# PaddlePaddle/PaddleScience

Measured on NVIDIA H100. Metric: collocation-points/sec PDE residual loss+grad (LDC N-S), higher is better.
Workload: dtype f32

## Files before the change

paddlescience_b200/csrc/kernels_wgmma.cuh:

```cuda
#pragma once

#include "kernels_thin.cuh"

#ifndef PPSCI_EMUL
#include <stdint.h>

namespace ppsci {
namespace wg {

constexpr int KCH = 32;
constexpr int THREADS = 256;
constexpr int TM = 64;
constexpr int A_TILE_BYTES = TM * KCH * 4;
__host__ __device__ inline int tile_points(int C) { return TM / C; }

__host__ __device__ inline int stage_bytes(int N) { return 2 * A_TILE_BYTES + 2 * N * KCH * 4; }
__host__ __device__ inline int fwd_smem_bytes(int N) { return 2 * stage_bytes(N) + 1024 + 64; }
constexpr int PREFETCH_MAX_CS = 8;

__host__ __device__ __forceinline__ uint32_t sw128(int row, int kk) {
  return (uint32_t)(row * 128 + ((((kk >> 2) ^ row) & 7) << 4) + ((kk & 3) << 2));
}
__device__ __forceinline__ uint32_t sw128_q(int row, int kq) { return (uint32_t)(row * 128 + (((kq ^ row) & 7) << 4)); }

__device__ __forceinline__ uint32_t smem_u32(const void* p) { return (uint32_t)__cvta_generic_to_shared(p); }

__device__ __forceinline__ float tf32_rn(float x) {
  uint32_t u;
  asm("cvt.rna.tf32.f32 %0, %1;" : "=r"(u) : "f"(x));
  return __uint_as_float(u);
}

__device__ __forceinline__ void mbar_init(uint32_t bar, uint32_t count) {
  asm volatile("mbarrier.init.shared::cta.b64 [%0], %1;" ::"r"(bar), "r"(count) : "memory");
}
__device__ __forceinline__ void mbar_expect_tx(uint32_t bar, uint32_t bytes) {
  asm volatile("mbarrier.arrive.expect_tx.shared::cta.b64 _, [%0], %1;" ::"r"(bar), "r"(bytes) : "memory");
}
__device__ __forceinline__ bool mbar_try_wait(uint32_t bar, uint32_t parity) {
  uint32_t ok;
  asm volatile(
      "{\n\t.reg .pred p;\n\t"
      "mbarrier.try_wait.parity.shared::cta.b64 p, [%1], %2;\n\t"
      "selp.u32 %0, 1, 0, p;\n\t}"
      : "=r"(ok)
      : "r"(bar), "r"(parity)
      : "memory");
  return ok != 0;
}
__device__ __forceinline__ void mbar_wait(uint32_t bar, uint32_t parity) {
  uint32_t spins = 0;
  while (!mbar_try_wait(bar, parity)) {
    if (++spins > (1u << 26)) __trap();
  }
}
__device__ __forceinline__ void bulk_g2s(uint32_t dst_smem, const void* src, uint32_t bytes, uint32_t bar) {
  asm volatile("cp.async.bulk.shared::cluster.global.mbarrier::complete_tx::bytes [%0], [%1], %2, [%3];" ::"r"(dst_smem),
               "l"(src), "r"(bytes), "r"(bar)
               : "memory");
}
__device__ __forceinline__ void fence_proxy_async() { asm volatile("fence.proxy.async.shared::cta;" ::: "memory"); }

__device__ __forceinline__ uint64_t make_desc(uint32_t saddr) {
  uint64_t d = 0;
  d |= (uint64_t)((saddr & 0x3FFFFu) >> 4);
  d |= (uint64_t)1 << 16;
  d |= (uint64_t)(1024 >> 4) << 32;
  d |= (uint64_t)1 << 62;
  return d;
}
__device__ __forceinline__ void wgmma_fence() { asm volatile("wgmma.fence.sync.aligned;" ::: "memory"); }
__device__ __forceinline__ void wgmma_commit() { asm volatile("wgmma.commit_group.sync.aligned;" ::: "memory"); }
template <int N>
__device__ __forceinline__ void wgmma_wait() {
  asm volatile("wgmma.wait_group.sync.aligned %0;" ::"n"(N) : "memory");
}
#define WG_T0 "%0, %1, %2, %3, %4, %5, %6, %7"
#define WG_T1 WG_T0 ", %8, %9, %10, %11, %12, %13, %14, %15"
#define WG_T2 WG_T1 ", %16, %17, %18, %19, %20, %21, %22, %23"
#define WG_T3 WG_T2 ", %24, %25, %26, %27, %28, %29, %30, %31"
#define WG_T4 WG_T3 ", %32, %33, %34, %35, %36, %37, %38, %39"
#define WG_T5 WG_T4 ", %40, %41, %42, %43, %44, %45, %46, %47"
#define WG_T6 WG_T5 ", %48, %49, %50, %51, %52, %53, %54, %55"
#define WG_T7 WG_T6 ", %56, %57, %58, %59, %60, %61, %62, %63"
#define WG_O8(b) "+f"(d[b]), "+f"(d[b + 1]), "+f"(d[b + 2]), "+f"(d[b + 3]), "+f"(d[b + 4]), "+f"(d[b + 5]), "+f"(d[b + 6]), "+f"(d[b + 7])
#define WG_O0 WG_O8(0)
#define WG_O1 WG_O0, WG_O8(8)
#define WG_O2 WG_O1, WG_O8(16)
#define WG_O3 WG_O2, WG_O8(24)
#define WG_O4 WG_O3, WG_O8(32)
#define WG_O5 WG_O4, WG_O8(40)
#define WG_O6 WG_O5, WG_O8(48)
#define WG_O7 WG_O6, WG_O8(56)
#define WG_MMA(M, G, IA, IB, IP)                                                                                  \
  __device__ __forceinline__ void wgmma_tf32(float (&d)[M / 2], uint64_t da, uint64_t db, uint32_t accumulate) { \
    asm volatile(                                                                                                 \
        "{\n\t.reg .pred p;\n\t"                                                                                  \
        "setp.ne.b32 p, %" #IP ", 0;\n\t"                                                                          \
        "wgmma.mma_async.sync.aligned.m64n" #M "k8.f32.tf32.tf32 {" WG_T##G "}, %" #IA ", %" #IB ", p, 1, 1;\n\t}"  \
        : WG_O##G                                                                                                 \
        : "l"(da), "l"(db), "r"(accumulate));                                                                     \
  }
WG_MMA(16, 0, 8, 9, 10)
WG_MMA(32, 1, 16, 17, 18)
WG_MMA(48, 2, 24, 25, 26)
WG_MMA(64, 3, 32, 33, 34)
WG_MMA(80, 4, 40, 41, 42)
WG_MMA(96, 5, 48, 49, 50)
WG_MMA(112, 6, 56, 57, 58)
WG_MMA(128, 7, 64, 65, 66)
#undef WG_MMA

__global__ void k_wg_prep_w(const float* __restrict__ W, float* __restrict__ img, int K, int N, int transposed) {
  const long long i = (long long)blockIdx.x * blockDim.x + threadIdx.x;
  if (i >= (long long)K * N) return;
  const int n = (int)(i / K), k = (int)(i % K);
  const float w = transposed ? W[(long long)n * K + k] : W[(long long)k * N + n];
  const float hi = tf32_rn(w);
  float* blk = img + (long long)(k / KCH) * 2 * N * KCH;
  const uint32_t off = sw128(n, k % KCH) >> 2;
  blk[off] = hi;
  blk[(long long)N * KCH + off] = w - hi;
}

struct WgArgs {
  AOperand<float> A;
  JetLayout J;
  const float* Wimg;
  int Kdim;
  int Kvalid;
  int Nout;
  const float* bias;
  float* Out;
  int ldo;
  long long oplane;
  long long Np;
  int num_tiles;
  const float* Zprev;
  int ldz;
  long long zplane;
  int act;
};

__device__ __forceinline__ unsigned char* xchg(unsigned char* base_ptr, int sbytes, int N, int r, int col) {
  return base_ptr + sbytes + 2 * A_TILE_BYTES + r * N * 4 + ((((col >> 2) ^ r) & 7) << 4) + (((col >> 2) & ~7) << 4) +
         (col & 3) * 4;
}

template <class L, int NQ, bool DX>
__global__ void __launch_bounds__(THREADS, 1) k_wg_layer(WgArgs g) {
  PPSCI_DYN_SMEM(smem_dyn);
  const uint32_t base = (smem_u32(smem_dyn) + 1023u) & ~1023u;
  unsigned char* base_ptr = smem_dyn + (base - smem_u32(smem_dyn));
  constexpr int CS = L::CS;
  constexpr int TP = TM / CS;
  constexpr int rows_used = CS * TP;
  constexpr int PPR = (THREADS / 32) * 4;
  constexpr int MAXI = (TP + PPR - 1) / PPR;
  constexpr int N = NQ * 32;
  constexpr int NH = N / 2;
  constexpr bool PREFETCH = CS <= PREFETCH_MAX_CS;
  const int sbytes = stage_bytes(N);
  const uint32_t bar0 = base + 2 * sbytes;
  const uint32_t b_bytes = (uint32_t)(2 * N * KCH * 4);
  const int tid = threadIdx.x, warp = tid >> 5, lane = tid & 31, wgi = tid >> 7;
  const int kq = lane & 7, psub = lane >> 3;
  const int nchunks = g.Kdim / KCH;
  const int act = g.A.act;

  if (tid == 0) {
    mbar_init(bar0, 1);
    mbar_init(bar0 + 8, 1);
    asm volatile("fence.mbarrier_init.release.cluster;" ::: "memory");
  }
  for (int s = 0; s < 2; ++s) {
    float4* az = reinterpret_cast<float4*>(base_ptr + s * sbytes);
    for (int i = tid; i < 2 * A_TILE_BYTES / 16; i += THREADS) az[i] = make_float4(0.f, 0.f, 0.f, 0.f);
  }
  fence_proxy_async();
  __syncthreads();

  float4 z[MAXI][CS];
  bool zok[MAXI];
  auto load_z = [&](int tile, int j) {
#pragma unroll
    for (int i = 0; i < MAXI; ++i) {
      const int pl = warp * 4 + psub + i * PPR;
      const long long p = (long long)tile * TP + pl;
      zok[i] = pl < TP && tile < g.num_tiles && p < g.Np;
      if (g.Kvalid && j * KCH + 4 * kq >= g.Kvalid) zok[i] = false;
      const float* src = g.A.Z + p * g.A.ld + j * KCH + 4 * kq;
#pragma unroll
      for (int c = 0; c < CS; ++c)
        z[i][c] = zok[i] ? __ldg(reinterpret_cast<const float4*>(src + (long long)c * g.A.plane)) : make_float4(0.f, 0.f, 0.f, 0.f);
    }
  };
  if constexpr (PREFETCH) load_z(blockIdx.x, 0);

  float ex[NH / 2], cr[NH / 2];
  const int rbase = (warp & 3) * 16 + (lane >> 2);
  const int cbase = wgi * NH + 2 * (lane & 3);
  uint32_t it = 0;
  for (int tile = blockIdx.x; tile < g.num_tiles; tile += gridDim.x) {
    const long long p0 = (long long)tile * TP;
#pragma unroll
    for (int e = 0; e < NH / 2; ++e) ex[e] = cr[e] = 0.f;
    for (int j = 0; j < nchunks; ++j, ++it) {
      const uint32_t s = it & 1u;
      wgmma_wait<1>();
      __syncthreads();
      const uint32_t st_addr = base + s * sbytes;
      unsigned char* st_ptr = base_ptr + s * sbytes;
      if (tid == 0) {
        mbar_expect_tx(bar0 + 8 * s, b_bytes);
        bulk_g2s(st_addr + 2 * A_TILE_BYTES, g.Wimg + (long long)j * 2 * N * KCH, b_bytes, bar0 + 8 * s);
      }
      if constexpr (!PREFETCH) load_z(tile, j);
#pragma unroll
      for (int i = 0; i < MAXI; ++i) {
        const int pl = warp * 4 + psub + i * PPR;
        if (pl >= TP) continue;
        const bool valid = zok[i];
        float yout[CS][4];
        if constexpr (DX) {
#pragma unroll
          for (int c = 0; c < CS; ++c) {
            yout[c][0] = z[i][c].x; yout[c][1] = z[i][c].y; yout[c][2] = z[i][c].z; yout[c][3] = z[i][c].w;
          }
        } else {
#pragma unroll
          for (int t = 0; t < 4; ++t) {
            auto comp = [&](const float4& v) { return t == 0 ? v.x : t == 1 ? v.y : t == 2 ? v.z : v.w; };
            float sc[6];
            float y0;
            act_coef<float, L::KM>(act, comp(z[i][0]), y0, sc);
            yout[0][t] = valid ? y0 : 0.f;
            jet_fwd<float, L>(g.J, sc, [&](int c) { return comp(z[i][c]); }, [&](int c, float v) { yout[c][t] = valid ? v : 0.f; });
          }
        }
#pragma unroll
        for (int c = 0; c < CS; ++c) {
          float4 h, l;
          h.x = tf32_rn(yout[c][0]); h.y = tf32_rn(yout[c][1]); h.z = tf32_rn(yout[c][2]); h.w = tf32_rn(yout[c][3]);
          l.x = yout[c][0] - h.x; l.y = yout[c][1] - h.y; l.z = yout[c][2] - h.z; l.w = yout[c][3] - h.w;
          const uint32_t off = sw128_q(c * TP + pl, kq);
          *reinterpret_cast<float4*>(st_ptr + off) = h;
          *reinterpret_cast<float4*>(st_ptr + A_TILE_BYTES + off) = l;
        }
      }
      if constexpr (PREFETCH) {
        if (j + 1 < nchunks) load_z(tile, j + 1);
        else load_z(tile + gridDim.x, 0);
      }
      fence_proxy_async();
      __syncthreads();
      mbar_wait(bar0 + 8 * s, (it >> 1) & 1u);
      const uint64_t a_hi = make_desc(st_addr), a_lo = make_desc(st_addr + A_TILE_BYTES);
      const uint64_t b_hi = make_desc(st_addr + 2 * A_TILE_BYTES + wgi * NH * 128), b_lo = b_hi + (uint64_t)(N * 128 / 16);
      wgmma_fence();
#pragma unroll
      for (int ks = 0; ks < KCH / 8; ++ks) {
        const uint64_t inc = (uint64_t)(2 * ks);
        const uint32_t first = (j == 0 && ks == 0) ? 0u : 1u;
        wgmma_tf32(ex, a_hi + inc, b_hi + inc, first);
        wgmma_tf32(cr, a_lo + inc, b_hi + inc, first);
        wgmma_tf32(cr, a_hi + inc, b_lo + inc, 1u);
      }
      wgmma_commit();
    }
    wgmma_wait<0>();
    if constexpr (!DX) {
#pragma unroll
      for (int h = 0; h < 2; ++h) {
        const int r = rbase + 8 * h;
        const int c = r / TP, pl = r - c * TP;
        const long long p = p0 + pl;
        if (r >= rows_used || p >= g.Np) continue;
        float* out_row = g.Out + (long long)c * g.oplane + p * g.ldo;
#pragma unroll
        for (int j = 0; j < NH / 8; ++j) {
          const int col = cbase + 8 * j;
          float2 v = make_float2(ex[4 * j + 2 * h] + cr[4 * j + 2 * h], ex[4 * j + 2 * h + 1] + cr[4 * j + 2 * h + 1]);
          if (c == 0 && g.bias) {
            v.x += __ldg(g.bias + col);
            v.y += __ldg(g.bias + col + 1);
          }
          *reinterpret_cast<float2*>(out_row + col) = v;
        }
      }
    } else {
      __syncthreads();
#pragma unroll
      for (int h = 0; h < 2; ++h) {
        const int r = rbase + 8 * h;
#pragma unroll
        for (int j = 0; j < NH / 8; ++j)
          *reinterpret_cast<float2*>(xchg(base_ptr, sbytes, N, r, cbase + 8 * j)) =
              make_float2(ex[4 * j + 2 * h] + cr[4 * j + 2 * h], ex[4 * j + 2 * h + 1] + cr[4 * j + 2 * h + 1]);
      }
      constexpr int N4 = N / 4;
      auto load_zc = [&](int item, float4 (&zc)[CS]) {
        const int pl = item / N4, q = item - pl * N4;
        const long long p = p0 + pl;
        if (item >= TP * N4 || p >= g.Np) return;
#pragma unroll
        for (int c = 0; c < CS; ++c)
          zc[c] = __ldg(reinterpret_cast<const float4*>(g.Zprev + (long long)c * g.zplane + p * g.ldz + 4 * q));
      };
      float4 znext[CS];
      if constexpr (PREFETCH) load_zc(tid, znext);
      __syncthreads();
      for (int item = tid; item < TP * N4; item += THREADS) {
        const int pl = item / N4, q = item - pl * N4;
        const long long p = p0 + pl;
        float4 zc[CS];
        if constexpr (PREFETCH) {
#pragma unroll
          for (int c = 0; c < CS; ++c) zc[c] = znext[c];
          load_zc(item + THREADS, znext);
        } else {
          load_zc(item, zc);
        }
        if (p >= g.Np) continue;
        float4 xc[CS];
#pragma unroll
        for (int c = 0; c < CS; ++c) xc[c] = *reinterpret_cast<const float4*>(xchg(base_ptr, sbytes, N, c * TP + pl, 4 * q));
        float ob[CS][4];
#pragma unroll
        for (int t = 0; t < 4; ++t) {
          auto comp = [&](const float4& v) { return t == 0 ? v.x : t == 1 ? v.y : t == 2 ? v.z : v.w; };
          float sc[6];
          float y0;
          act_coef<float, L::KM + 1>(g.act, comp(zc[0]), y0, sc);
          ob[0][t] = jet_adj<float, L>(g.J, sc, [&](int c) { return comp(zc[c]); }, [&](int c) { return comp(xc[c]); },
                                       [&](int c, float v) { ob[c][t] = v; });
        }
        float* out = g.Out + p * g.ldo + 4 * q;
#pragma unroll
        for (int c = 0; c < CS; ++c)
          *reinterpret_cast<float4*>(out + (long long)c * g.oplane) = make_float4(ob[c][0], ob[c][1], ob[c][2], ob[c][3]);
      }
      fence_proxy_async();
      __syncthreads();
    }
  }
}

__host__ __device__ constexpr int dw_pch(int C) { return C >= 8 ? 4 : C >= 3 ? 8 : 32 / C; }
__host__ __device__ constexpr int dw_groups(int C) { return dw_pch(C) / 4 * C; }
__host__ __device__ constexpr int dw_ksteps(int C) { return (dw_groups(C) + 1) / 2; }
__host__ __device__ constexpr int dw_atoms(int C) { return (dw_ksteps(C) + 3) / 4; }
__host__ __device__ constexpr int dw_maxq(int C) { return C <= 5 ? 4 : C <= 8 ? 2 : 1; }
__host__ __device__ constexpr int dw_smem_bytes(int C, int bnq) {
  return 2 * 2 * dw_atoms(C) * bnq * 32 * 128 + bnq * 32 * 4 + dw_pch(C) / 4 * 2 * C * 256 * 4 + bnq * 32 * 2 * 256 + 1024;
}
constexpr int DW_TK = 128;
constexpr int DW_FLUSH_ROWS = 512;
__host__ __device__ constexpr int dw_flush(int C) {
  return DW_FLUSH_ROWS / (dw_pch(C) * C) > 1 ? DW_FLUSH_ROWS / (dw_pch(C) * C) : 1;
}

struct WgDwArgs {
  AOperand<float> A;
  JetLayout J;
  const float* Zbar;
  int ldzb;
  long long zbplane;
  int Kdim;
  int Nout;
  int col_blocks;
  float* dW;
  float* db;
  long long Np;
  int chunks_per_split;
};

__device__ __forceinline__ void wgmma_tf32_rA_m64n64(float (&d)[32], const uint32_t (&a)[4], uint64_t db) {
  asm volatile(
      "{\n\t.reg .pred p;\n\t"
      "setp.ne.b32 p, %37, 0;\n\t"
      "wgmma.mma_async.sync.aligned.m64n64k8.f32.tf32.tf32 "
      "{%0, %1, %2, %3, %4, %5, %6, %7, %8, %9, %10, %11, %12, %13, %14, %15, "
      "%16, %17, %18, %19, %20, %21, %22, %23, %24, %25, %26, %27, %28, %29, %30, %31}, "
      "{%32, %33, %34, %35}, %36, p, 1, 1;\n\t}"
      : "+f"(d[0]), "+f"(d[1]), "+f"(d[2]), "+f"(d[3]), "+f"(d[4]), "+f"(d[5]), "+f"(d[6]), "+f"(d[7]), "+f"(d[8]),
        "+f"(d[9]), "+f"(d[10]), "+f"(d[11]), "+f"(d[12]), "+f"(d[13]), "+f"(d[14]), "+f"(d[15]), "+f"(d[16]),
        "+f"(d[17]), "+f"(d[18]), "+f"(d[19]), "+f"(d[20]), "+f"(d[21]), "+f"(d[22]), "+f"(d[23]), "+f"(d[24]),
        "+f"(d[25]), "+f"(d[26]), "+f"(d[27]), "+f"(d[28]), "+f"(d[29]), "+f"(d[30]), "+f"(d[31])
      : "r"(a[0]), "r"(a[1]), "r"(a[2]), "r"(a[3]), "l"(db), "r"(1u));
}
__device__ __forceinline__ void wgmma_tf32_rA_m64n32(float (&d)[16], const uint32_t (&a)[4], uint64_t db) {
  asm volatile(
      "{\n\t.reg .pred p;\n\t"
      "setp.ne.b32 p, %21, 0;\n\t"
      "wgmma.mma_async.sync.aligned.m64n32k8.f32.tf32.tf32 "
      "{%0, %1, %2, %3, %4, %5, %6, %7, %8, %9, %10, %11, %12, %13, %14, %15}, "
      "{%16, %17, %18, %19}, %20, p, 1, 1;\n\t}"
      : "+f"(d[0]), "+f"(d[1]), "+f"(d[2]), "+f"(d[3]), "+f"(d[4]), "+f"(d[5]), "+f"(d[6]), "+f"(d[7]), "+f"(d[8]),
        "+f"(d[9]), "+f"(d[10]), "+f"(d[11]), "+f"(d[12]), "+f"(d[13]), "+f"(d[14]), "+f"(d[15])
      : "r"(a[0]), "r"(a[1]), "r"(a[2]), "r"(a[3]), "l"(db), "r"(1u));
}

template <class L, int BNQ>
__global__ void __launch_bounds__(THREADS, 1) k_wg_dw(WgDwArgs g) {
  PPSCI_DYN_SMEM(smem_dyn);
  const uint32_t base = (smem_u32(smem_dyn) + 1023u) & ~1023u;
  unsigned char* base_ptr = smem_dyn + (base - smem_u32(smem_dyn));
  constexpr int CS = L::CS, PCH = dw_pch(CS), QPC = PCH / 4, G = dw_groups(CS), KS = dw_ksteps(CS), NA = dw_atoms(CS);
  constexpr int BN = BNQ * 32, NB = BNQ / 2, TAIL = BNQ & 1;
  constexpr int ATOM = BN * 128;
  constexpr int STAGE = 2 * NA * ATOM;
  constexpr int BI = (G * BN + THREADS - 1) / THREADS;
  const int tid = threadIdx.x, warp = tid >> 5, lane = tid & 31, wgi = tid >> 7, t = lane & 3;
  const int kb = blockIdx.x / g.col_blocks, n0 = (blockIdx.x - kb * g.col_blocks) * BN;
  const int Np = (int)g.Np;
  const int total_chunks = (Np + PCH - 1) / PCH;
  const int ch_begin = blockIdx.y * g.chunks_per_split;
  const int ch_end = ch_begin + g.chunks_per_split < total_chunks ? ch_begin + g.chunks_per_split : total_chunks;
  if (ch_begin >= ch_end) return;
  const int act = g.A.act;
  const int krow = kb * DW_TK + wgi * 64 + (warp & 3) * 16 + (lane >> 2);

  float* bsum = reinterpret_cast<float*>(base_ptr + 2 * STAGE);
  for (int i = tid; i < (2 * STAGE + BN * 4) / 16; i += THREADS)
    reinterpret_cast<float4*>(base_ptr)[i] = make_float4(0.f, 0.f, 0.f, 0.f);
  __syncthreads();

  float ex[NB > 0 ? NB : 1][32], ext[TAIL ? 16 : 1], cr[NB > 0 ? NB : 1][32], crt[TAIL ? 16 : 1];
#pragma unroll
  for (int nb = 0; nb < NB; ++nb)
#pragma unroll
    for (int i = 0; i < 32; ++i) ex[nb][i] = cr[nb][i] = 0.f;
#pragma unroll
  for (int i = 0; i < (TAIL ? 16 : 1); ++i) ext[i] = crt[i] = 0.f;

  auto acc_at = [&](int e) -> float {
    return e < 32 * NB ? ex[e >> 5][e & 31] + cr[e >> 5][e & 31] : ext[e - 32 * NB] + crt[e - 32 * NB];
  };
  float4* part = reinterpret_cast<float4*>(base_ptr + 2 * STAGE + BN * 4 + QPC * 2 * CS * THREADS * 4);
#pragma unroll
  for (int q = 0; q < BN / 8; ++q) part[q * THREADS + tid] = make_float4(0.f, 0.f, 0.f, 0.f);
  auto flush = [&]() {
#pragma unroll
    for (int q = 0; q < BN / 8; ++q) {
      float4 p = part[q * THREADS + tid];
      p.x += acc_at(4 * q); p.y += acc_at(4 * q + 1); p.z += acc_at(4 * q + 2); p.w += acc_at(4 * q + 3);
      part[q * THREADS + tid] = p;
    }
#pragma unroll
    for (int nb = 0; nb < NB; ++nb)
#pragma unroll
      for (int i = 0; i < 32; ++i) ex[nb][i] = cr[nb][i] = 0.f;
#pragma unroll
    for (int i = 0; i < (TAIL ? 16 : 1); ++i) ext[i] = crt[i] = 0.f;
  };

  float* za = reinterpret_cast<float*>(base_ptr + 2 * STAGE + BN * 4);
  auto za_at = [&](int qq, int h, int c) -> float* { return za + ((qq * 2 + h) * CS + c) * THREADS + tid; };
  float4 zb[BI];
  auto load_a = [&](int ch) {
    const int p0 = ch * PCH;
#pragma unroll
    for (int qq = 0; qq < QPC; ++qq)
#pragma unroll
      for (int h = 0; h < 2; ++h) {
        const int p = p0 + 4 * qq + t;
        const int k = krow + 8 * h;
        const bool ok = p < Np && k < g.Kdim;
        const float* src = g.A.Z + (ok ? (long long)p * g.A.ld + k : 0);
#pragma unroll
        for (int c = 0; c < CS; ++c)
          asm volatile("cp.async.ca.shared.global [%0], [%1], 4, %2;" ::"r"(smem_u32(za_at(qq, h, c))),
                       "l"(src + (ok ? (long long)c * g.A.plane : 0)), "r"(ok ? 4 : 0)
                       : "memory");
      }
    asm volatile("cp.async.commit_group;" ::: "memory");
  };
  auto load_b = [&](int ch) {
    const int p0 = ch * PCH;
#pragma unroll
    for (int i = 0; i < BI; ++i) {
      const int item = tid + THREADS * i;
      const int gi = item / BN, n = item - gi * BN;
      const int qq = gi / CS, c = gi - qq * CS;
      const int p = p0 + 4 * qq;
      const bool ok = item < G * BN && n0 + n < g.Nout;
      const float* src = g.Zbar + (long long)c * g.zbplane + (long long)p * g.ldzb + n0 + n;
      zb[i].x = ok && p < Np ? __ldg(src) : 0.f;
      zb[i].y = ok && p + 1 < Np ? __ldg(src + g.ldzb) : 0.f;
      zb[i].z = ok && p + 2 < Np ? __ldg(src + 2 * g.ldzb) : 0.f;
      zb[i].w = ok && p + 3 < Np ? __ldg(src + 3 * g.ldzb) : 0.f;
    }
  };

  load_a(ch_begin);
  load_b(ch_begin);
  uint32_t ahi[KS][4], alo[KS][4];
  for (int ch = ch_begin; ch < ch_end; ++ch) {
    const int sidx = (ch - ch_begin) & 1;
    const uint32_t st_addr = base + sidx * STAGE;
    unsigned char* st = base_ptr + sidx * STAGE;
#pragma unroll
    for (int i = 0; i < BI; ++i) {
      const int item = tid + THREADS * i;
      if (item >= G * BN) continue;
      const int gi = item / BN, n = item - gi * BN;
      const float4 v = zb[i];
      float4 hi, lo;
      hi.x = tf32_rn(v.x); hi.y = tf32_rn(v.y); hi.z = tf32_rn(v.z); hi.w = tf32_rn(v.w);
      lo.x = v.x - hi.x; lo.y = v.y - hi.y; lo.z = v.z - hi.z; lo.w = v.w - hi.w;
      const uint32_t off = (gi >> 3) * ATOM + sw128_q(n, gi & 7);
      *reinterpret_cast<float4*>(st + off) = hi;
      *reinterpret_cast<float4*>(st + NA * ATOM + off) = lo;
      if (kb == 0 && gi % CS == 0) atomicAdd(bsum + n, (v.x + v.y) + (v.z + v.w));
    }
    wgmma_wait<0>();
    if (ch > ch_begin && (ch - ch_begin) % dw_flush(CS) == 0) flush();
    asm volatile("cp.async.wait_group 0;" ::: "memory");
    float av[QPC][2][CS];
#pragma unroll
    for (int qq = 0; qq < QPC; ++qq)
#pragma unroll
      for (int h = 0; h < 2; ++h) {
        float z[CS], sc[6];
#pragma unroll
        for (int c = 0; c < CS; ++c) z[c] = *za_at(qq, h, c);
        act_coef<float, L::KM>(act, z[0], av[qq][h][0], sc);
        jet_fwd<float, L>(g.J, sc, [&](int c) { return z[c]; }, [&](int c, float v) { av[qq][h][c] = v; });
      }
    if (ch + 1 < ch_end) load_a(ch + 1);
    fence_proxy_async();
    __syncthreads();
    if (ch + 1 < ch_end) load_b(ch + 1);
#pragma unroll
    for (int s = 0; s < KS; ++s)
#pragma unroll
      for (int e = 0; e < 2; ++e)
#pragma unroll
        for (int h = 0; h < 2; ++h) {
          const int gi = 2 * s + e;
          const float v = gi < G ? av[gi / CS][h][gi % CS] : 0.f;
          const float vh = tf32_rn(v);
          ahi[s][2 * e + h] = __float_as_uint(vh);
          alo[s][2 * e + h] = __float_as_uint(v - vh);
        }
    wgmma_fence();
#pragma unroll
    for (int s = 0; s < KS; ++s) {
      const uint64_t b_hi = make_desc(st_addr + (s >> 2) * ATOM + (s & 3) * 32);
      const uint64_t b_lo = b_hi + (uint64_t)(NA * ATOM / 16);
#pragma unroll
      for (int nb = 0; nb < NB; ++nb) {
        const uint64_t bo = (uint64_t)(nb * 64 * 128 / 16);
        wgmma_tf32_rA_m64n64(ex[nb], ahi[s], b_hi + bo);
        wgmma_tf32_rA_m64n64(cr[nb], alo[s], b_hi + bo);
        wgmma_tf32_rA_m64n64(cr[nb], ahi[s], b_lo + bo);
      }
      if constexpr (TAIL) {
        const uint64_t bo = (uint64_t)(NB * 64 * 128 / 16);
        wgmma_tf32_rA_m64n32(ext, ahi[s], b_hi + bo);
        wgmma_tf32_rA_m64n32(crt, alo[s], b_hi + bo);
        wgmma_tf32_rA_m64n32(crt, ahi[s], b_lo + bo);
      }
    }
    wgmma_commit();
  }
  wgmma_wait<0>();
#pragma unroll
  for (int h = 0; h < 2; ++h) {
    const int k = krow + 8 * h;
    if (k >= g.Kdim) continue;
    float* row = g.dW + (long long)k * g.Nout + n0;
#pragma unroll
    for (int j = 0; j < BN / 8; ++j) {
      if (n0 + 8 * j >= g.Nout) break;
      const int col = 8 * j + 2 * t;
      const float4 p = part[j * THREADS + tid];
      atomicAdd(row + col, (h ? p.z : p.x) + acc_at(4 * j + 2 * h));
      atomicAdd(row + col + 1, (h ? p.w : p.y) + acc_at(4 * j + 2 * h + 1));
    }
  }
  if (kb == 0) {
    __syncthreads();
    if (tid < BN && n0 + tid < g.Nout) atomicAdd(g.db + n0 + tid, bsum[tid]);
  }
}

}

inline int wg_kpad(int K) { return (K + wg::KCH - 1) / wg::KCH * wg::KCH; }
inline bool wg_shape_ok(int K, int N) { return K % wg::KCH == 0 && K >= 32 && K <= 1024 && N % 32 == 0 && N >= 32 && N <= 256; }
inline bool wg_plan_ok(const ppsci_plan_spec& s, const JetLayout& J) {
  return s.dtype == PPSCI_F32 && !s.gated && !act_has_param(s.act) && with_lay(WgLays{}, J, [](auto) {});
}
inline bool wg_fwd_ok(const ppsci_plan_spec& s, int l) {
  if (l == 1) return s.dense_in && s.n_layers >= 2 && s.widths[0] % 4 == 0 && wg_shape_ok(wg_kpad(s.widths[0]), s.widths[1]);
  if (l < 2 || l > s.n_layers) return false;
  return wg_shape_ok(s.widths[l - 1], s.widths[l]);
}
inline bool wg_dx_ok(const ppsci_plan_spec& s, int l) {
  if (l < 2 || l > s.n_layers) return false;
  return wg_shape_ok(s.widths[l], s.widths[l - 1]);
}

inline bool wg_dw_ok(const ppsci_plan_spec& s, int l) {
  if (l < 1 || (l == 1 && !s.dense_in) || l > s.n_layers) return false;
  const int K = s.widths[l - 1], N = s.widths[l];
  return K % 4 == 0 && N % 32 == 0 && N >= 32 && N <= 256;
}

}
#endif
```

Measured before the change: 5.996 million.

## Decouple weight staging into triple-buffered ring prefetched one chunk ahead

Splits shared memory so the A-operand tiles keep a two-stage buffer while the weight (B) tiles get their own three-slot ring with three mbarriers. The bulk copy for the next K-chunk (or the next tile's first chunk) is issued one iteration ahead, so the weight load overlaps the A-tile conversion and the previous wgmma instead of being fetched and waited on within the same iteration. The DX exchange scratch now lives in the free ring slot. This costs one extra B stage of shared memory, which may limit larger N, and the slot and parity arithmetic is more delicate.

Result: faster. 6.068 million, median of 6 (+1.2%).

```diff
diff --git a/paddlescience_b200/csrc/kernels_wgmma.cuh b/paddlescience_b200/csrc/kernels_wgmma.cuh
--- a/paddlescience_b200/csrc/kernels_wgmma.cuh
+++ b/paddlescience_b200/csrc/kernels_wgmma.cuh
@@ -14,8 +14,9 @@
 constexpr int A_TILE_BYTES = TM * KCH * 4;
 __host__ __device__ inline int tile_points(int C) { return TM / C; }
 
-__host__ __device__ inline int stage_bytes(int N) { return 2 * A_TILE_BYTES + 2 * N * KCH * 4; }
-__host__ __device__ inline int fwd_smem_bytes(int N) { return 2 * stage_bytes(N) + 1024 + 64; }
+constexpr int A_STAGE_BYTES = 2 * A_TILE_BYTES;
+__host__ __device__ inline int b_stage_bytes(int N) { return 2 * N * KCH * 4; }
+__host__ __device__ inline int fwd_smem_bytes(int N) { return 2 * A_STAGE_BYTES + 3 * b_stage_bytes(N) + 1024 + 64; }
 constexpr int PREFETCH_MAX_CS = 8;
 
 __host__ __device__ __forceinline__ uint32_t sw128(int row, int kk) {
@@ -142,9 +143,8 @@
   int act;
 };
 
-__device__ __forceinline__ unsigned char* xchg(unsigned char* base_ptr, int sbytes, int N, int r, int col) {
-  return base_ptr + sbytes + 2 * A_TILE_BYTES + r * N * 4 + ((((col >> 2) ^ r) & 7) << 4) + (((col >> 2) & ~7) << 4) +
-         (col & 3) * 4;
+__device__ __forceinline__ unsigned char* xchg(unsigned char* xb, int N, int r, int col) {
+  return xb + r * N * 4 + ((((col >> 2) ^ r) & 7) << 4) + (((col >> 2) & ~7) << 4) + (col & 3) * 4;
 }
 
 template <class L, int NQ, bool DX>
@@ -160,9 +160,9 @@
   constexpr int N = NQ * 32;
   constexpr int NH = N / 2;
   constexpr bool PREFETCH = CS <= PREFETCH_MAX_CS;
-  const int sbytes = stage_bytes(N);
-  const uint32_t bar0 = base + 2 * sbytes;
-  const uint32_t b_bytes = (uint32_t)(2 * N * KCH * 4);
+  constexpr uint32_t b_bytes = (uint32_t)(2 * N * KCH * 4);
+  const uint32_t bbase = base + 2 * A_STAGE_BYTES;
+  const uint32_t bar0 = bbase + 3 * b_bytes;
   const int tid = threadIdx.x, warp = tid >> 5, lane = tid & 31, wgi = tid >> 7;
   const int kq = lane & 7, psub = lane >> 3;
   const int nchunks = g.Kdim / KCH;
@@ -171,14 +171,19 @@
   if (tid == 0) {
     mbar_init(bar0, 1);
     mbar_init(bar0 + 8, 1);
+    mbar_init(bar0 + 16, 1);
     asm volatile("fence.mbarrier_init.release.cluster;" ::: "memory");
   }
   for (int s = 0; s < 2; ++s) {
-    float4* az = reinterpret_cast<float4*>(base_ptr + s * sbytes);
+    float4* az = reinterpret_cast<float4*>(base_ptr + s * A_STAGE_BYTES);
     for (int i = tid; i < 2 * A_TILE_BYTES / 16; i += THREADS) az[i] = make_float4(0.f, 0.f, 0.f, 0.f);
   }
   fence_proxy_async();
   __syncthreads();
+  if (tid == 0 && (int)blockIdx.x < g.num_tiles) {
+    mbar_expect_tx(bar0, b_bytes);
+    bulk_g2s(bbase, g.Wimg, b_bytes, bar0);
+  }
 
   float4 z[MAXI][CS];
   bool zok[MAXI];
@@ -206,14 +211,15 @@
 #pragma unroll
     for (int e = 0; e < NH / 2; ++e) ex[e] = cr[e] = 0.f;
     for (int j = 0; j < nchunks; ++j, ++it) {
-      const uint32_t s = it & 1u;
+      const uint32_t s = it & 1u, sb = it % 3u;
       wgmma_wait<1>();
       __syncthreads();
-      const uint32_t st_addr = base + s * sbytes;
-      unsigned char* st_ptr = base_ptr + s * sbytes;
-      if (tid == 0) {
-        mbar_expect_tx(bar0 + 8 * s, b_bytes);
-        bulk_g2s(st_addr + 2 * A_TILE_BYTES, g.Wimg + (long long)j * 2 * N * KCH, b_bytes, bar0 + 8 * s);
+      const uint32_t st_addr = base + s * A_STAGE_BYTES;
+      unsigned char* st_ptr = base_ptr + s * A_STAGE_BYTES;
+      if (tid == 0 && (j + 1 < nchunks || tile + (int)gridDim.x < g.num_tiles)) {
+        const uint32_t nb = sb == 2u ? 0u : sb + 1u;
+        mbar_expect_tx(bar0 + 8 * nb, b_bytes);
+        bulk_g2s(bbase + nb * b_bytes, g.Wimg + (long long)(j + 1 < nchunks ? j + 1 : 0) * 2 * N * KCH, b_bytes, bar0 + 8 * nb);
       }
       if constexpr (!PREFETCH) load_z(tile, j);
 #pragma unroll
@@ -254,9 +260,9 @@
       }
       fence_proxy_async();
       __syncthreads();
-      mbar_wait(bar0 + 8 * s, (it >> 1) & 1u);
+      mbar_wait(bar0 + 8 * sb, (it / 3u) & 1u);
       const uint64_t a_hi = make_desc(st_addr), a_lo = make_desc(st_addr + A_TILE_BYTES);
-      const uint64_t b_hi = make_desc(st_addr + 2 * A_TILE_BYTES + wgi * NH * 128), b_lo = b_hi + (uint64_t)(N * 128 / 16);
+      const uint64_t b_hi = make_desc(bbase + sb * b_bytes + wgi * NH * 128), b_lo = b_hi + (uint64_t)(N * 128 / 16);
       wgmma_fence();
 #pragma unroll
       for (int ks = 0; ks < KCH / 8; ++ks) {
@@ -290,12 +296,13 @@
       }
     } else {
       __syncthreads();
+      unsigned char* xb = base_ptr + 2 * A_STAGE_BYTES + ((it + 1u) % 3u) * b_bytes;
 #pragma unroll
       for (int h = 0; h < 2; ++h) {
         const int r = rbase + 8 * h;
 #pragma unroll
         for (int j = 0; j < NH / 8; ++j)
-          *reinterpret_cast<float2*>(xchg(base_ptr, sbytes, N, r, cbase + 8 * j)) =
+          *reinterpret_cast<float2*>(xchg(xb, N, r, cbase + 8 * j)) =
               make_float2(ex[4 * j + 2 * h] + cr[4 * j + 2 * h], ex[4 * j + 2 * h + 1] + cr[4 * j + 2 * h + 1]);
       }
       constexpr int N4 = N / 4;
@@ -324,7 +331,7 @@
         if (p >= g.Np) continue;
         float4 xc[CS];
 #pragma unroll
-        for (int c = 0; c < CS; ++c) xc[c] = *reinterpret_cast<const float4*>(xchg(base_ptr, sbytes, N, c * TP + pl, 4 * q));
+        for (int c = 0; c < CS; ++c) xc[c] = *reinterpret_cast<const float4*>(xchg(xb, N, c * TP + pl, 4 * q));
         float ob[CS][4];
 #pragma unroll
         for (int t = 0; t < 4; ++t) {
```
